# Gautham-JS/ROS_Stereo_SLAM

Hardware: AMD Instinct MI355X
Metric: stereo frames/sec @1241x376, 4096 kpts (higher is better)
Workload: dtype u8/i32 fixed-point (LK) + f32/f64 (geometry)

## Files before the change

### include/svo.h

```cpp
#ifndef SVO_H
#define SVO_H

#include <stddef.h>
#include <stdint.h>

#ifdef __cplusplus
extern "C" {
#endif

#define SVO_VERSION 100

enum {
    SVO_OK = 0,
    SVO_ERR_ARG = -1,
    SVO_ERR_HIP = -2,
    SVO_ERR_CAPACITY = -3,
    SVO_ERR_NO_DEVICE = -4,
    SVO_ERR_TRACKING_LOST = -5,
    SVO_ERR_STATE = -6
};
enum { SVO_MEM_HOST = 0, SVO_MEM_DEVICE = 1 };

enum {
    SVO_K_PYRAMID = 0,
    SVO_K_LK = 1,
    SVO_K_FRANSAC = 2,
    SVO_K_TRIANGULATE = 3,
    SVO_K_PNP = 4,
    SVO_K_POSEGRAPH = 5,
    SVO_K_ANMS = 6,
    SVO_K_BRIEF_INTEGRAL = 7,
    SVO_K_BRIEF_DESCRIBE = 8,
    SVO_K_COUNT = 9
};

typedef struct svo_ctx svo_ctx;
typedef struct svo_pyramid svo_pyramid;
typedef struct svo_vo svo_vo;
typedef struct svo_posegraph svo_posegraph;

int svo_version(void);
const char *svo_last_error(void);

int svo_ctx_create(int device, svo_ctx **out);
int svo_ctx_destroy(svo_ctx *ctx);
int svo_ctx_sync(svo_ctx *ctx);
void *svo_ctx_stream(svo_ctx *ctx);
int svo_ctx_enable_kernel_timing(svo_ctx *ctx, int enable);
int svo_ctx_kernel_time(svo_ctx *ctx, int kernel_id, double *total_ms, int *launches);
int svo_ctx_reset_kernel_time(svo_ctx *ctx);

enum { SVO_MATH_SIN = 0, SVO_MATH_COS = 1, SVO_MATH_ACOS = 2, SVO_MATH_CBRT = 3, SVO_MATH_LOG = 4, SVO_MATH_EXP = 5 };
int svo_math_eval(svo_ctx *ctx, int fn, const double *x, int n, double *y, int mem);

int svo_selftest_fransac_gate(svo_ctx *ctx, const float *d_p1, const float *d_p2, int n, double threshold,
                              uint64_t seed, int lean, uint8_t *d_mask, unsigned *tickets_after);
enum { SVO_SCAN_256_INT = 0, SVO_SCAN_1024_UINT = 1, SVO_SCAN_1024_U64 = 2 };
int svo_selftest_scan(svo_ctx *ctx, int kind, const void *d_in, int n, void *d_out, void *d_total);

int svo_pyramid_create(svo_ctx *ctx, int width, int height, int channels, int levels,
                       svo_pyramid **out);
int svo_pyramid_destroy(svo_ctx *ctx, svo_pyramid *pyr);
int svo_pyramid_build(svo_ctx *ctx, svo_pyramid *pyr, const uint8_t *image, int mem);
int svo_pyramid_is_mono(svo_ctx *ctx, const svo_pyramid *pyr, int *out);
int svo_pyramid_get_level(svo_ctx *ctx, const svo_pyramid *pyr, int level, uint8_t *out,
                          int mem, int *w, int *h);
int svo_pyramid_create2(svo_ctx *ctx, int width, int height, int channels, int levels, int want_deriv,
                        svo_pyramid **out);
int svo_pyramid_get_padded_level(svo_ctx *ctx, const svo_pyramid *pyr, int level, uint8_t *out, int mem,
                                 int *pw, int *ph);
int svo_pyramid_get_derivative_level(svo_ctx *ctx, const svo_pyramid *pyr, int level, int32_t *out, int mem,
                                     int *pw, int *ph);

int svo_grid_keypoints(svo_ctx *ctx, int rows, int cols, int step, float *out_xy, int cap,
                       int mem, int *count);

int svo_lk_track(svo_ctx *ctx, const svo_pyramid *prev, const svo_pyramid *next,
                 const float *prev_pts, int n, float *next_pts, uint8_t *status, float *err,
                 float *min_eig, int mem);

int svo_lk_track_jobs(svo_ctx *ctx, int n_jobs, svo_pyramid *const *prev, const svo_pyramid *const *next,
                      const float *const *d_prev_pts, const int *n, float *const *d_next_pts, uint8_t *const *d_status,
                      float *const *d_err, float *const *d_min_eig, const int *const *d_gates);
int svo_pyramid_build_gated(svo_ctx *ctx, svo_pyramid *pyr, const uint8_t *d_image, const int *d_gate);
int svo_pyramid_build_many(svo_ctx *ctx, int k, svo_pyramid *const *pyrs, const uint8_t *const *d_images,
                           const int *const *d_gates);

int svo_compact(svo_ctx *ctx, const uint8_t *mask, int n, const float *in_a, int stride_a, float *out_a,
                const float *in_b, int stride_b, float *out_b, const float *in_c, int stride_c, float *out_c,
                int *count, int mem);

int svo_fransac(svo_ctx *ctx, const float *p1, const float *p2, int n, double threshold,
                double confidence, int max_iters, uint64_t seed, uint8_t *mask, double *F9,
                int *inlier_count, int *iters_run, int mem);
typedef struct svo_fransac_problem {
    const float *p1, *p2;
    int cap;
    const int *d_n;
    double threshold, confidence;
    int max_iters;
    uint64_t seed;
    uint8_t *mask;
    double *F9;
    int *inlier_count, *iters_run;
    const float *payload_in[3];
    float *payload_out[3];
    int payload_stride[3];
    int *payload_count;
    const int *gate;
} svo_fransac_problem;
int svo_fransac_batch(svo_ctx *ctx, int k, const svo_fransac_problem *problems);

int svo_stereo_projections(double fx, double fy, double cx, double cy, double baseline, double *P1,
                           double *P2);
int svo_triangulate(svo_ctx *ctx, const double *P1, const double *P2, const float *x1, const float *x2,
                    int n, float *out_xyz, float *out_h4, int mem);
int svo_transform_points(svo_ctx *ctx, const double *Rt, const float *in_xyz, int n, float *out_xyz,
                         int mem);
int svo_get_colors(svo_ctx *ctx, const svo_pyramid *pyr, const float *xy, int n, float *out_bgr, int mem);

#define SVO_DEDUP_BOX  0
#define SVO_DEDUP_DISC 1
int svo_dedup_points(svo_ctx *ctx, const float *ref_xy, int n_ref, const int *ref_idx, int n_idx, const float *new_xy,
                     int n_new, double radius, int mode, uint8_t *keep, int *n_keep, int mem);
int svo_replenish(svo_ctx *ctx, float *ref_xy, float *ref_xyz, int n_ref, int cap, const float *new_xy, const float *new_xyz,
// ... 452 lines not shown
```

### ros_stereo_slam_amd/csrc/pyramid.hip

```cpp
#include <cstdlib>

#include "pyr_grey_plan.hip.h"
#include "svo_internal.h"

namespace {

namespace pgp = pyr_grey_plan;

__device__ __forceinline__ int reflect101(int p, int len)
{
    if (len == 1)
        return 0;
    while (p < 0 || p >= len)
        p = p < 0 ? -p : 2 * (len - 1) - p;
    return p;
}

constexpr int TW = 32, TH = 8;
constexpr int PB = 64;
constexpr int SW = 2 * TW + 3, SH = 2 * TH + 3;
constexpr int ROWS_PER_BLOCK = 8;
constexpr int PYR_JOBS = 2 * SVO_LK_MAX_JOBS;

template <int NJ> struct PyrBuildN {
    const uint8_t *img[NJ];
    uint8_t *lvl[NJ][SVO_MAX_LEVELS];
    int *dlvl[NJ];
    const int *gate[NJ];
    int doff[SVO_MAX_LEVELS];
    int pitch[SVO_MAX_LEVELS], dpitch[SVO_MAX_LEVELS], w[SVO_MAX_LEVELS], h[SVO_MAX_LEVELS];
    int levels;
    int gdelta[SVO_MAX_LEVELS], gdoff[SVO_MAX_LEVELS];
    int storage;
};
using PyrBuild = PyrBuildN<PYR_JOBS>;
constexpr int PYR_FEW = 2;
inline PyrBuildN<PYR_FEW> pyr_few(const PyrBuild &b)
{
    PyrBuildN<PYR_FEW> f;
    for (int a = 0; a < PYR_FEW; a++) {
        f.img[a] = b.img[a];
        for (int l = 0; l < SVO_MAX_LEVELS; l++)
            f.lvl[a][l] = b.lvl[a][l];
        f.dlvl[a] = b.dlvl[a];
        f.gate[a] = b.gate[a];
    }
    for (int l = 0; l < SVO_MAX_LEVELS; l++) {
        f.doff[l] = b.doff[l];
        f.pitch[l] = b.pitch[l];
        f.dpitch[l] = b.dpitch[l];
        f.w[l] = b.w[l];
        f.h[l] = b.h[l];
        f.gdelta[l] = b.gdelta[l];
        f.gdoff[l] = b.gdoff[l];
    }
    f.levels = b.levels;
    f.storage = b.storage;
    return f;
}
static_assert(sizeof(PyrBuild) <= 3072, "kernel arguments are limited to 4 KB");
static_assert(pgp::PAD == SVO_PYR_PAD && pgp::LANES == PB && pgp::TILE_W == TW && pgp::TILE_H == TH && pgp::SRC_W == SW &&
                  pgp::SRC_H == SH,
              "pyr_grey_plan.hip.h restates these");

template <int C, bool RAW, int SC = C>
__device__ __forceinline__ void down_tile(const uint8_t *__restrict__ src, int spitch, int w, int h,
                                          uint8_t *__restrict__ dst, int dpitch, int dw, int dh, int tx, int ty)
{
    constexpr int ND = (SW * C + 3) / 4;
    constexpr int SROW = (ND + 1) * 4;
    constexpr int VROW = ND * 4 + 4;
    __shared__ __attribute__((aligned(16))) uint8_t s_src[SH * SROW];
    __shared__ __attribute__((aligned(16))) uint16_t s_v[TH][VROW];
    const int tid = threadIdx.x;
    const int ox = tx * TW, oy = ty * TH;
    const int x0 = 2 * ox - 2, y0 = 2 * oy - 2;
    const bool interior = SC == C && x0 >= 0 && x0 + SW <= w && y0 >= 0 && y0 + SH <= h &&
                          (!RAW || (size_t)(y0 + SH - 1) * spitch + (size_t)x0 * C + (ND + 1) * 4 + 4 <= (size_t)h * spitch);
    bool grey_interior = false;
    if constexpr (RAW && C == 1 && SC == 3) {
        static_assert(ND == pgp::SRC_ND, "the staged row of pyr_grey_plan.hip.h");
        grey_interior = pgp::l1_tile_interior(src, w, h, x0, y0);
    }
    if (grey_interior) {
        if constexpr (RAW && C == 1 && SC == 3) {
            uint32_t staged[pgp::L1_TURNS];
#pragma unroll
            for (int turn = 0; turn < pgp::L1_TURNS; turn++) {
                const int i = min(turn * PB + tid, pgp::L1_ITEMS - 1);
                staged[turn] = pgp::l1_stage_item(src, w, x0, y0, i / ND, i % ND);
            }
#pragma unroll
            for (int turn = 0; turn < pgp::L1_TURNS; turn++) {
                const int i = turn * PB + tid;
                if (i < pgp::L1_ITEMS)
                    reinterpret_cast<uint32_t *>(s_src + (i / ND) * SROW)[i % ND] = staged[turn];
            }
        }
    } else if (interior) {
        for (int d = tid; d < ND; d += PB) {
            const uint8_t *col = src + (ptrdiff_t)y0 * spitch + x0 * C;
#pragma unroll 1
            for (int r = 0; r < SH; r++) {
                const uint8_t *row = col + (ptrdiff_t)r * spitch;
                const unsigned sh = (unsigned)(reinterpret_cast<uintptr_t>(row) & 3);
                const uint32_t *p = reinterpret_cast<const uint32_t *>(row - sh) + d;
                reinterpret_cast<uint32_t *>(s_src + r * SROW)[d] = __builtin_amdgcn_alignbyte(p[1], p[0], sh);
            }
        }
    } else {
        for (int d = tid; d < ND; d += PB) {
            int sx[4];
#pragma unroll
// ... 179 lines not shown

template <int C, int NJ> __global__ __launch_bounds__(PB) void pyr_down_kernel(PyrBuildN<NJ> b, int l)
{
    svo_chain_priority();
    const int job = blockIdx.z;
    if (b.gate[job] && *b.gate[job] == 0)
        return;
    if constexpr (C == 3) {
        if (__builtin_amdgcn_readfirstlane(pyr_words_of(b, job, C)[SVO_PYR_STORED]) == 1) {
            down_tile<1, false>(b.lvl[job][l - 1] + b.gdelta[l - 1], svo_grey_pitch(b.w[l - 1]), b.w[l - 1], b.h[l - 1],
                                b.lvl[job][l] + b.gdelta[l], svo_grey_pitch(b.w[l]), b.w[l], b.h[l], blockIdx.x, blockIdx.y);
            return;
        }
    }
    down_tile<C, false>(b.lvl[job][l - 1], b.pitch[l - 1], b.w[l - 1], b.h[l - 1], b.lvl[job][l], b.pitch[l],
                        b.w[l], b.h[l], blockIdx.x, blockIdx.y);
}

template <int C>
__device__ __forceinline__ void fill_border_row(uint8_t *__restrict__ level, int w, int h, int pitch, int row, int d)
{
    const bool interior_row = row >= SVO_PYR_PAD && row < SVO_PYR_PAD + h;
    const int cb0 = d * 4;
    if (interior_row && cb0 >= SVO_PYR_PAD * C && cb0 + 3 < (SVO_PYR_PAD + w) * C)
        return;
    uint8_t *prow = level + (size_t)row * pitch;
    const int Y = reflect101(row - SVO_PYR_PAD, h);
    const uint8_t *srow = level + (size_t)(Y + SVO_PYR_PAD) * pitch + SVO_PYR_PAD * C;
#pragma unroll
    for (int b = 0; b < 4; b++) {
        int cb = cb0 + b;
        int px = cb / C, ch = cb - px * C;
        bool inside = interior_row && px >= SVO_PYR_PAD && px < SVO_PYR_PAD + w;
        if (inside)
            continue;
        uint8_t v = 0;
        if (px < w + 2 * SVO_PYR_PAD)
            v = srow[reflect101(px - SVO_PYR_PAD, w) * C + ch];
        prow[cb] = v;
    }
}

template <int C> __device__ __forceinline__ bool scharr_edge(int w, int q) { return q == 0 || 4 * q + 4 + C > w * C; }
template <int C> __device__ __forceinline__ void scharr_edge_offsets(int w, int q, int (&off)[12])
{
#pragma unroll
    for (int i = 0; i < 12; i++) {
        const int cb = 4 * q - 4 + i;
        const int px = cb >= 0 ? cb / C : -((-cb + C - 1) / C);
        off[i] = reflect101(px, w) * C + (cb - px * C);
    }
}

template <int C>
__device__ __forceinline__ void scharr_row(const uint8_t *__restrict__ lvl, int *__restrict__ dlvl, int pitch, int dpitch,
                                           int w, int h, int y, int q, const int (&edge_off)[12])
{
    const uint8_t *rows[3] = {lvl + (ptrdiff_t)reflect101(y - 1, h) * pitch, lvl + (ptrdiff_t)y * pitch,
                              lvl + (ptrdiff_t)reflect101(y + 1, h) * pitch};
    uint32_t win[3][3];
    if (!scharr_edge<C>(w, q)) {
#pragma unroll
        for (int r = 0; r < 3; r++) {
            const uint32_t *p = reinterpret_cast<const uint32_t *>(rows[r]) + (q - 1);
            win[r][0] = p[0];
            win[r][1] = p[1];
            win[r][2] = p[2];
        }
    } else {
#pragma unroll
        for (int r = 0; r < 3; r++)
#pragma unroll
            for (int d = 0; d < 3; d++) {
                uint32_t v = 0;
#pragma unroll
                for (int bb = 0; bb < 4; bb++)
                    v |= (uint32_t)rows[r][edge_off[4 * d + bb]] << (8 * bb);
                win[r][d] = v;
            }
    }
    typedef short short2v __attribute__((ext_vector_type(2)));
    short2v S[6], V[6];
#pragma unroll
    for (int k = 0; k < 6; k++) {
        const unsigned sel = (k & 1) ? 0x0c030c02u : 0x0c010c00u;
        const short2v a = __builtin_bit_cast(short2v, __builtin_amdgcn_perm(0u, win[0][k >> 1], sel));
        const short2v bq = __builtin_bit_cast(short2v, __builtin_amdgcn_perm(0u, win[1][k >> 1], sel));
        const short2v c = __builtin_bit_cast(short2v, __builtin_amdgcn_perm(0u, win[2][k >> 1], sel));
        const short2v three = {3, 3}, ten = {10, 10};
        S[k] = (a + c) * three + bq * ten;
        V[k] = c - a;
    }
    auto pair_at = [](const short2v (&P)[6], int pos) -> short2v {
        if ((pos & 1) == 0)
            return P[pos >> 1];
        return __builtin_bit_cast(short2v, __builtin_amdgcn_perm(__builtin_bit_cast(unsigned, P[(pos >> 1) + 1]),
                                                                 __builtin_bit_cast(unsigned, P[pos >> 1]), 0x05040302u));
    };
    int out[4];
#pragma unroll
    for (int j = 0; j < 4; j += 2) {
        const short2v four = {4, 4}, twelve = {12, 12}, forty = {40, 40};
        const short2v dx = (pair_at(S, 4 + C + j) - pair_at(S, 4 - C + j)) * four;
        const short2v dy = (pair_at(V, 4 - C + j) + pair_at(V, 4 + C + j)) * twelve + pair_at(V, 4 + j) * forty;
        const unsigned ux = __builtin_bit_cast(unsigned, dx), uy = __builtin_bit_cast(unsigned, dy);
        out[j] = (int)__builtin_amdgcn_perm(uy, ux, 0x05040100u);
        out[j + 1] = (int)__builtin_amdgcn_perm(uy, ux, 0x07060302u);
    }
    int *drow = reinterpret_cast<int *>(reinterpret_cast<uint8_t *>(dlvl) + (ptrdiff_t)y * dpitch);
    const int rem = w * C - 4 * q;
    if (rem >= 4) {
        typedef int int4v __attribute__((ext_vector_type(4)));
        *reinterpret_cast<int4v *>(drow + 4 * q) = int4v{out[0], out[1], out[2], out[3]};
    } else {
        for (int j = 0; j < rem; j++)
            drow[4 * q + j] = out[j];
    }
}

struct FinishPlan {
    int border_y0[SVO_MAX_LEVELS + 1];
    int scharr_y0[SVO_MAX_LEVELS + 1];
    int publish;
};
template <int S, int NJ, class Pitch, class DPitch>
__device__ __forceinline__ void finish_roles(const PyrBuildN<NJ> &b, const FinishPlan &plan, int job, int by, const int (&ldelta)[SVO_MAX_LEVELS],
                                             const int (&ldoff)[SVO_MAX_LEVELS], Pitch pitch, DPitch dpitch)
{
    if (by < plan.border_y0[b.levels]) {
        int l = 1;
        for (int i = 2; i < b.levels; i++)
            l = by >= plan.border_y0[i] ? i : l;
        const int d = blockIdx.x * PB + threadIdx.x;
        if (d >= (pitch(l) >> 2))
            return;
        uint8_t *padded = b.lvl[job][l] + ldelta[l] - (size_t)SVO_PYR_PAD * pitch(l) - SVO_PYR_PAD * S;
        for (int row = (by - plan.border_y0[l]) * ROWS_PER_BLOCK, rend = min(row + ROWS_PER_BLOCK, b.h[l] + 2 * SVO_PYR_PAD);
             row < rend; row++)
            fill_border_row<S>(padded, b.w[l], b.h[l], pitch(l), row, d);
        return;
    }
    if (!b.dlvl[job])
        return;
    int l = 0;
    for (int i = 1; i < b.levels; i++)
        l = by >= plan.scharr_y0[i] ? i : l;
    const int q = blockIdx.x * PB + threadIdx.x;
    if (4 * q >= b.w[l] * S)
        return;
    int edge_off[12] = {0, 0, 0, 0, 0, 0, 0, 0, 0, 0, 0, 0};
    if (scharr_edge<S>(b.w[l], q))
        scharr_edge_offsets<S>(b.w[l], q, edge_off);
    for (int y = (by - plan.scharr_y0[l]) * ROWS_PER_BLOCK, yend = min(y + ROWS_PER_BLOCK, b.h[l]); y < yend; y++)
        scharr_row<S>(b.lvl[job][l] + ldelta[l], b.dlvl[job] + ldoff[l], pitch(l), dpitch(l), b.w[l], b.h[l], y, q, edge_off);
}

template <int C, int NJ> __global__ __launch_bounds__(PB) void pyr_finish_kernel(PyrBuildN<NJ> b, FinishPlan plan)
{
    svo_chain_priority();
    const int job = blockIdx.z, by = blockIdx.y;
    if (b.gate[job] && *b.gate[job] == 0)
        return;
    if constexpr (C == 3) {
        int *words = pyr_words_of(b, job, C);
        const bool grey = __builtin_amdgcn_readfirstlane(words[SVO_PYR_STORED]) == 1;
        if (blockIdx.x == 0 && by == 0 && threadIdx.x == 0) {
            if (plan.publish) {
                words[SVO_PYR_MONO] = words[SVO_PYR_COLOUR_SEEN] == 0;
                words[SVO_PYR_COLOUR_SEEN] = 0;
                words[SVO_PYR_COLOUR_VALID] = 0;
            } else {
                words[SVO_PYR_COLOUR_VALID] &= ~2;
            }
        }
        if (grey) {
            finish_roles<1>(b, plan, job, by, b.gdelta, b.gdoff, [&](int l) { return svo_grey_pitch(b.w[l]); },
                            [&](int l) { return svo_grey_dpitch(b.w[l]); });
            return;
        }
    }
    const int zero[SVO_MAX_LEVELS] = {0, 0, 0, 0};
    finish_roles<C>(b, plan, job, by, zero, b.doff, [&](int l) { return b.pitch[l]; }, [&](int l) { return b.dpitch[l]; });
}

}

static int alloc_derivative_levels(svo_ctx *ctx, svo_pyramid *p)
{
    size_t ints = 0;
    for (int l = 0; l < p->levels; l++) {
        p->dpitch[l] = (((p->dev.w[l] + 2 * SVO_DERIV_PAD) * p->c * 4 + 15) / 16) * 16;
        const size_t lvl_ints = (size_t)(p->dpitch[l] / 4) * (p->dev.h[l] + 2 * SVO_DERIV_PAD);
        p->doff[l] = ints + (size_t)SVO_DERIV_PAD * (p->dpitch[l] / 4) + (size_t)SVO_DERIV_PAD * p->c;
        ints += (lvl_ints + 63) & ~(size_t)63;
    }
    if (p->c == 3)
        for (int l = 0; l < p->levels; l++) {
            const int gdp = svo_grey_dpitch(p->dev.w[l]);
            p->gdoff[l] = ints + (size_t)SVO_DERIV_PAD * (gdp / 4) + (size_t)SVO_DERIV_PAD;
            ints += ((size_t)(gdp / 4) * (p->dev.h[l] + 2 * SVO_DERIV_PAD) + 63) & ~(size_t)63;
        }
    const size_t dbytes = ints * 4 + 1024;
    hipError_t e = hipMalloc((void **)&p->dbase, dbytes);
    if (e == hipSuccess)
        e = hipMemsetAsync(p->dbase, 0, dbytes, ctx->stream);
    if (e != hipSuccess) {
        (void)hipFree(p->dbase);
        p->dbase = nullptr;
        svo_set_error("hipMalloc derivative levels -> %s", hipGetErrorString(e));
        return SVO_ERR_HIP;
    }
    return SVO_OK;
}

static void fill_build(PyrBuild &b, int k, svo_pyramid *const *pyrs, const uint8_t *const *d_images, bool deriv_only,
                       const int *const *gates = nullptr)
{
    for (int a = 0; a < PYR_JOBS; a++)
        b.gate[a] = gates ? gates[a < k ? a : 0] : nullptr;
    const svo_pyramid *p0 = pyrs[0];
    for (int l = 0; l < SVO_MAX_LEVELS; l++) {
        b.pitch[l] = p0->dev.pitch[l];
        b.w[l] = p0->dev.w[l];
        b.h[l] = p0->dev.h[l];
        b.dpitch[l] = 0;
        b.doff[l] = 0;
        b.gdelta[l] = p0->gdelta[l];
        b.gdoff[l] = 0;
    }
    b.levels = p0->levels;
    static const int mono_storage = getenv("SVO_PYR_MONO_STORAGE") ? atoi(getenv("SVO_PYR_MONO_STORAGE")) : 1;
    b.storage = mono_storage;
    for (int a = 0; a < PYR_JOBS; a++) {
        svo_pyramid *p = pyrs[a < k ? a : 0];
        b.img[a] = d_images ? d_images[a < k ? a : 0] : nullptr;
        for (int l = 0; l < SVO_MAX_LEVELS; l++)
            b.lvl[a][l] = l < p->levels ? const_cast<uint8_t *>(p->dev.lvl[l]) : nullptr;
        const bool d = p->dbase && (deriv_only || p->want_deriv) && (p->c == 1 || p->c == 3);
        b.dlvl[a] = d ? p->dbase : nullptr;
        if (d)
            for (int l = 0; l < SVO_MAX_LEVELS; l++) {
                b.dpitch[l] = p->dpitch[l];
                b.doff[l] = (int)p->doff[l];
                b.gdoff[l] = (int)p->gdoff[l];
            }
    }
}

template <int C> static int launch_finish(svo_ctx *ctx, int k, const PyrBuild &b, bool borders)
{
    FinishPlan plan;
    int y = 0, xmax = 1;
    for (int l = 0; l <= SVO_MAX_LEVELS; l++)
        plan.border_y0[l] = plan.scharr_y0[l] = 0;
    for (int l = 1; l < b.levels; l++) {
        plan.border_y0[l] = y;
        if (borders) {
            y += (b.h[l] + 2 * SVO_PYR_PAD + ROWS_PER_BLOCK - 1) / ROWS_PER_BLOCK;
            xmax = max(xmax, ((b.pitch[l] >> 2) + PB - 1) / PB);
        }
    }
    for (int l = b.levels; l <= SVO_MAX_LEVELS; l++)
        plan.border_y0[l] = y;
    plan.border_y0[b.levels] = y;
    bool any_deriv = false;
    for (int a = 0; a < k; a++)
        any_deriv = any_deriv || b.dlvl[a];
    for (int l = 0; l < b.levels; l++) {
        plan.scharr_y0[l] = y;
        if (any_deriv) {
            y += (b.h[l] + ROWS_PER_BLOCK - 1) / ROWS_PER_BLOCK;
            xmax = max(xmax, ((b.w[l] * C + 3) / 4 + PB - 1) / PB);
        }
    }
    plan.scharr_y0[b.levels] = y;
    plan.publish = borders ? 1 : 0;
    if (y == 0)
        return SVO_OK;
    if (k <= PYR_FEW)
        hipLaunchKernelGGL((pyr_finish_kernel<C, PYR_FEW>), dim3(xmax, y, k), dim3(PB), 0, ctx->stream, pyr_few(b), plan);
    else
        hipLaunchKernelGGL((pyr_finish_kernel<C, PYR_JOBS>), dim3(xmax, y, k), dim3(PB), 0, ctx->stream, b, plan);
    SVO_HIP(hipGetLastError());
    return SVO_OK;
}

int svo_build_derivatives(svo_ctx *ctx, int k, svo_pyramid *const *pyrs)
{
    if (k <= 0)
        return SVO_OK;
    if (k > PYR_JOBS) {
        svo_set_error("pyramid: at most %d per launch", PYR_JOBS);
        return SVO_ERR_ARG;
    }
    for (int a = 0; a < k; a++)
        if (pyrs[a]->c != 1 && pyrs[a]->c != 3) {
            svo_set_error("pyramid: %d channels carry no derivative levels", pyrs[a]->c);
            return SVO_ERR_STATE;
        }
    for (int a = 0; a < k; a++)
        if (!pyrs[a]->dbase) {
            SVO_HIP(hipSetDevice(ctx->device));
            const int rc = alloc_derivative_levels(ctx, pyrs[a]);
            if (rc)
                return rc;
        }
    PyrBuild b;
    fill_build(b, k, pyrs, nullptr, true);
    const int rc = pyrs[0]->c == 1 ? launch_finish<1>(ctx, k, b, false) : launch_finish<3>(ctx, k, b, false);
    if (rc == SVO_OK)
        for (int a = 0; a < k; a++)
            pyrs[a]->has_deriv = true;
    return rc;
}

template <int C>
static int build_levels(svo_ctx *ctx, int k, svo_pyramid *const *pyrs, const uint8_t *const *d_images, const int *const *gates)
{
    PyrBuild b;
    fill_build(b, k, pyrs, d_images, false, gates);
    if constexpr (C == 3) {
        const int quads = (b.w[0] * b.h[0] + 3) / 4, gx = (quads + PB * HEAD_TURNS - 1) / (PB * HEAD_TURNS);
        if (k <= PYR_FEW)
            hipLaunchKernelGGL((pyr_head_kernel<PYR_FEW>), dim3(gx, k), dim3(PB), 0, ctx->stream, pyr_few(b));
        else
            hipLaunchKernelGGL((pyr_head_kernel<PYR_JOBS>), dim3(gx, k), dim3(PB), 0, ctx->stream, b);
    }
    {
        const int tiles_x = b.levels > 1 ? (b.w[1] + TW - 1) / TW : 0, tiles_y = b.levels > 1 ? (b.h[1] + TH - 1) / TH : 0;
        const int n_tiles = tiles_x * tiles_y;
        const int pad_x = ((b.pitch[0] >> 2) + PB - 1) / PB,
                  pad_y = (b.h[0] + 2 * SVO_PYR_PAD + ROWS_PER_BLOCK - 1) / ROWS_PER_BLOCK;
        if (k <= PYR_FEW)
            hipLaunchKernelGGL((pyr_base_kernel<C, PYR_FEW>), dim3(n_tiles + pad_x * pad_y, k), dim3(PB), 0, ctx->stream,
                               pyr_few(b), tiles_x > 0 ? tiles_x : 1, n_tiles, pad_x);
// ... 211 lines not shown
    return svo_pyramid_create_ex(ctx, width, height, channels, levels, want_deriv != 0, out);
}

int svo_pyramid_get_padded_level(svo_ctx *ctx, const svo_pyramid *pyr, int level, uint8_t *out, int mem, int *pw, int *ph)
{
    SVO_CHECK_ARG(ctx && pyr && level >= 0 && level < pyr->levels);
    SVO_CHECK_ARG(mem == SVO_MEM_HOST || mem == SVO_MEM_DEVICE);
    const int W = pyr->dev.w[level] + 2 * SVO_PYR_PAD, H = pyr->dev.h[level] + 2 * SVO_PYR_PAD;
    if (pw)
        *pw = W;
    if (ph)
        *ph = H;
    if (out) {
        const int rc = svo_expand_grey_storage(ctx, pyr, false);
        if (rc)
            return rc;
        const size_t rowb = (size_t)W * pyr->c;
        SVO_HIP(hipMemcpy2DAsync(out, rowb, pyr->base + pyr->off[level], pyr->dev.pitch[level], rowb, H,
                                 mem == SVO_MEM_HOST ? hipMemcpyDeviceToHost : hipMemcpyDeviceToDevice, ctx->stream));
        if (mem == SVO_MEM_HOST)
            SVO_HIP(hipStreamSynchronize(ctx->stream));
    }
    return SVO_OK;
}

int svo_pyramid_get_derivative_level(svo_ctx *ctx, const svo_pyramid *pyr, int level, int32_t *out, int mem, int *pw, int *ph)
{
    SVO_CHECK_ARG(ctx && pyr && level >= 0 && level < pyr->levels);
    SVO_CHECK_ARG(mem == SVO_MEM_HOST || mem == SVO_MEM_DEVICE);
    if (!pyr->dbase || !pyr->has_deriv || (pyr->c != 1 && pyr->c != 3)) {
        svo_set_error("pyramid: holds no derivative levels");
        return SVO_ERR_STATE;
    }
    const int W = pyr->dev.w[level] + 2 * SVO_DERIV_PAD, H = pyr->dev.h[level] + 2 * SVO_DERIV_PAD;
    if (pw)
        *pw = W;
    if (ph)
        *ph = H;
    if (out) {
        const int rc = svo_expand_grey_storage(ctx, pyr, true);
        if (rc)
            return rc;
        const size_t rowb = (size_t)W * pyr->c * sizeof(int32_t);
        const int *first = pyr->dbase + pyr->doff[level] - (size_t)SVO_DERIV_PAD * (pyr->dpitch[level] / 4) -
                           (size_t)SVO_DERIV_PAD * pyr->c;
        SVO_HIP(hipMemcpy2DAsync(out, rowb, first, pyr->dpitch[level], rowb, H,
                                 mem == SVO_MEM_HOST ? hipMemcpyDeviceToHost : hipMemcpyDeviceToDevice, ctx->stream));
        if (mem == SVO_MEM_HOST)
            SVO_HIP(hipStreamSynchronize(ctx->stream));
    }
    return SVO_OK;
}

int svo_pyramid_build_many(svo_ctx *ctx, int k, svo_pyramid *const *pyrs, const uint8_t *const *d_images,
                           const int *const *d_gates)
{
    SVO_CHECK_ARG(ctx && k >= 1 && k <= PYR_JOBS && pyrs && d_images);
    for (int a = 0; a < k; a++)
        SVO_CHECK_ARG(pyrs[a] && d_images[a]);
    return svo_build_pyramids_from_device(ctx, k, pyrs, d_images, d_gates);
}

}
```

### ros_stereo_slam_amd/csrc/svo_internal.h

```cpp
#pragma once

#include <hip/hip_runtime.h>

#include <cstdint>
#include <cstdio>
#include <cstring>
#include <string>
#include <vector>

#include "../../include/svo.h"
#include "../../include/svo_math.h"

#define SVO_MAX_LEVELS 4
#define SVO_LK_WIN 21
#define SVO_PYR_PAD 32
#define SVO_LK_MAX_JOBS 16

#define SVO_N_TICKETS 64
static_assert(32 + 2 * SVO_LK_MAX_JOBS <= SVO_N_TICKETS, "svo_ctx::d_tickets: lk_expand_kernel's slots end past the allocation");

void svo_set_error(const char *fmt, ...);

__device__ __forceinline__ void svo_chain_priority() { __builtin_amdgcn_s_setprio(3); }

// ... 17 lines not shown
    } while (0)

struct PyrDev {
    const uint8_t *lvl[SVO_MAX_LEVELS];
    int pitch[SVO_MAX_LEVELS];
    int w[SVO_MAX_LEVELS];
    int h[SVO_MAX_LEVELS];
    int levels;
    int c;
};

struct Mat34 {
    double m[12];
};

#define SVO_PYR_HEADER 256
enum { SVO_PYR_MONO = 0, SVO_PYR_COLOUR_SEEN = 1, SVO_PYR_STORED = 2, SVO_PYR_COLOUR_VALID = 3 };
__host__ __device__ __forceinline__ int *svo_pyr_words(const uint8_t *padded)
{
    return reinterpret_cast<int *>(const_cast<uint8_t *>(padded) - SVO_PYR_HEADER);
}
__host__ __device__ __forceinline__ int svo_grey_pitch(int w) { return (w + 2 * SVO_PYR_PAD + 15) & ~15; }
__host__ __device__ __forceinline__ int svo_grey_dpitch(int w) { return ((w + 2 * 32 ) * 4 + 15) & ~15; }
__device__ __forceinline__ const uint8_t *svo_pyr_pixel0(const uint8_t *lvl0, int pitch, int c, int w, int gdelta0, int x, int y,
                                                         int *step)
{
    *step = c >= 3 ? 1 : 0;
    if (c == 3) {
        const int *words = svo_pyr_words(lvl0 - (ptrdiff_t)SVO_PYR_PAD * pitch - SVO_PYR_PAD * c);
        if (words[SVO_PYR_STORED] == 1) {
            *step = 0;
            return lvl0 + gdelta0 + (ptrdiff_t)y * svo_grey_pitch(w) + x;
        }
    }
    return lvl0 + (size_t)y * pitch + x * c;
}

struct svo_pyramid {
    int w, h, c, levels;
    uint8_t *base;
    size_t off[SVO_MAX_LEVELS];
    uint8_t *origin(int l) const
    {
        return base + off[l] + (size_t)SVO_PYR_PAD * dev.pitch[l] + (size_t)SVO_PYR_PAD * c;
    }
    size_t bytes;
    PyrDev dev;
    int *dbase = nullptr;
    size_t doff[SVO_MAX_LEVELS] = {0, 0, 0, 0};
    int dpitch[SVO_MAX_LEVELS] = {0, 0, 0, 0};
    size_t goff[SVO_MAX_LEVELS] = {0, 0, 0, 0}, gdoff[SVO_MAX_LEVELS] = {0, 0, 0, 0};
    int gdelta[SVO_MAX_LEVELS] = {0, 0, 0, 0};
    bool want_deriv = true, has_deriv = false;
};
#define SVO_DERIV_PAD 32
int svo_build_derivatives(svo_ctx *ctx, int k, svo_pyramid *const *pyrs);
int svo_expand_grey_storage(svo_ctx *ctx, const svo_pyramid *pyr, bool deriv);
int svo_pyramid_create_ex(svo_ctx *ctx, int width, int height, int channels, int levels, bool want_deriv,
                          svo_pyramid **out);

struct DevBuf {
    void *p = nullptr;
    size_t cap = 0;
    int ensure(size_t bytes);
    void release();
    template <class T> T *as() { return reinterpret_cast<T *>(p); }
};

struct KernelTimer {
    std::vector<std::pair<hipEvent_t, hipEvent_t>> pending;
    std::vector<std::pair<hipEvent_t, hipEvent_t>> pool;
    double total_ms = 0;
    int launches = 0;
};

struct svo_ctx {
    int device = 0;
    hipStream_t stream = nullptr;
    bool timing = false;
    KernelTimer timers[SVO_K_COUNT];
    DevBuf s_img, s_a, s_b, s_c, s_d, s_e, s_f, s_g;
    DevBuf w_a, w_b, w_c, w_d, w_e;
    unsigned *d_tickets = nullptr;
    void *pinned = nullptr;
    size_t pinned_bytes = 0;
    hipEvent_t wait_ev = nullptr;
    struct svo_orb *orb_cache = nullptr;
    int orb_key[5] = {0, 0, 0, 0, 0};
    DevBuf orb_out;
    std::vector<unsigned char> orb_host;
    struct svo_orb_cv *orb_cv_cache = nullptr;
    int orb_cv_key[8] = {0, 0, 0, 0, 0, 0, 0, 0};
    int8_t orb_pattern[1024];
    int has_pattern = 0;
    DevBuf orb_cv_out, orb_cv_img, orb_cv_ptrs;
    hipStream_t up_stream = nullptr;
    DevBuf up_ring;
    hipEvent_t up_ev[3] = {nullptr, nullptr, nullptr}, use_ev[3] = {nullptr, nullptr, nullptr};
    DevBuf sgbm_cost, sgbm_misc, sgbm_rp;
    DevBuf bm_work;
    DevBuf sor_grid;
    DevBuf icp_work;
    DevBuf ess;
    DevBuf feat_img, feat_sum;
    DevBuf sift_pyr, sift_work, sift_out;
    DevBuf brief_work, brief_pat;
// ... 220 lines not shown
```

Measured before the change: 14670.

## Flatten pyramid finish kernel into a balanced 1D work-item schedule with row-reuse Scharr

Replaces the 3D grid (x blocks × per-level row bands × jobs) of the pyramid finish kernel with a 1D grid. A host-built plan packs border-fill and Scharr items per job and spreads them evenly across workgroups, and grey-stored pyramids pick a row granularity that fits the same workgroup count. The Scharr pass now processes several rows per thread with a rolling three-row window, so each source row is loaded once instead of three times. This is meant to remove idle blocks in the old rectangular grid and redundant loads, at the cost of a larger kernel argument and per-item decode logic. The change also adds a small public accessor for a pyramid's device memory regions.

```diff
diff --git a/include/svo.h b/include/svo.h
--- a/include/svo.h
+++ b/include/svo.h
@@ -71,6 +71,7 @@
                                  int *pw, int *ph);
 int svo_pyramid_get_derivative_level(svo_ctx *ctx, const svo_pyramid *pyr, int level, int32_t *out, int mem,
                                      int *pw, int *ph);
+int svo_pyramid_device_regions(const svo_pyramid *pyr, void **base, size_t *bytes, void **dbase, size_t *dbytes);
 
 int svo_grid_keypoints(svo_ctx *ctx, int rows, int cols, int step, float *out_xy, int cap,
                        int mem, int *count);
diff --git a/ros_stereo_slam_amd/csrc/pyr_finish_plan.hip.h b/ros_stereo_slam_amd/csrc/pyr_finish_plan.hip.h
--- /dev/null
+++ b/ros_stereo_slam_amd/csrc/pyr_finish_plan.hip.h
@@ -0,0 +1,140 @@
+#pragma once
+
+#if defined(__HIPCC__)
+#define PYR_FINISH_HD __host__ __device__ inline __attribute__((always_inline))
+#else
+#define PYR_FINISH_HD inline
+#endif
+
+namespace pyr_finish_plan {
+
+constexpr int PAD = 32;
+constexpr int LANES = 64;
+constexpr int MAX_LEVELS = 4;
+constexpr int MAX_JOBS = 32;
+constexpr int ROWS = 8;
+enum { BORDER = 0, SCHARR = 1 };
+
+struct Table {
+    int S;
+    int rows;
+    int n[2];
+    int start[2][MAX_LEVELS];
+    int xb[2][MAX_LEVELS];
+    int ext_x[2][MAX_LEVELS];
+    int ext_rows[2][MAX_LEVELS];
+};
+
+struct Item {
+    int role, level;
+    int row0, nrows;
+    int x0, nx;
+};
+
+struct Plan {
+    Table full, grey;
+    int has_grey;
+    int k, nd;
+    int nbw, nsw;
+    unsigned dmask;
+    int publish;
+    unsigned char djob[MAX_JOBS];
+};
+
+PYR_FINISH_HD int pitch_of(int w, int S) { return ((w + 2 * PAD) * S + 15) / 16 * 16; }
+PYR_FINISH_HD int ceil_div(int a, int b) { return (a + b - 1) / b; }
+
+inline Table make_table(int levels, const int *w, const int *h, int S, int rows, bool borders, bool scharr)
+{
+    Table t;
+    t.S = S;
+    t.rows = rows;
+    for (int role = 0; role < 2; role++) {
+        int n = 0;
+        for (int l = 0; l < MAX_LEVELS; l++) {
+            const bool has = l < levels && (role == BORDER ? borders && l >= 1 : scharr);
+            t.start[role][l] = n;
+            t.ext_x[role][l] = !has ? 0 : role == BORDER ? pitch_of(w[l], S) / 4 : (w[l] * S + 3) / 4;
+            t.ext_rows[role][l] = !has ? 0 : role == BORDER ? h[l] + 2 * PAD : h[l];
+            t.xb[role][l] = has ? ceil_div(t.ext_x[role][l], LANES) : 1;
+            n += has ? t.xb[role][l] * ceil_div(t.ext_rows[role][l], rows) : 0;
+        }
+        t.n[role] = n;
+    }
+    return t;
+}
+
+PYR_FINISH_HD int job_items(const Table &t, bool deriv) { return t.n[BORDER] + (deriv ? t.n[SCHARR] : 0); }
+PYR_FINISH_HD int job_wgs(const Plan &p, bool deriv) { return p.nbw + (deriv ? p.nsw : 0); }
+PYR_FINISH_HD int grid_wgs(const Plan &p) { return p.k * p.nbw + p.nd * p.nsw; }
+
+inline Plan make_plan(int levels, const int *w, const int *h, int C, bool borders, int k, const bool *deriv)
+{
+    Plan p;
+    p.k = k;
+    p.nd = 0;
+    p.dmask = 0;
+    p.publish = borders ? 1 : 0;
+    for (int a = 0; a < MAX_JOBS; a++)
+        p.djob[a] = 0;
+    for (int a = 0; a < k; a++)
+        if (deriv[a]) {
+            p.dmask |= 1u << a;
+            p.djob[p.nd++] = (unsigned char)a;
+        }
+    p.full = make_table(levels, w, h, C, ROWS, borders, p.nd > 0);
+    p.nsw = p.full.n[SCHARR];
+    p.nbw = p.full.n[BORDER];
+    if (borders && p.nbw == 0 && p.nsw > 0)
+        p.nbw = 1;
+    p.has_grey = C == 3;
+    p.grey = p.full;
+    if (p.has_grey)
+        for (int rows = 1; rows <= ROWS; rows++) {
+            p.grey = make_table(levels, w, h, 1, rows, borders, p.nd > 0);
+            if (job_items(p.grey, false) <= job_wgs(p, false) && (p.nd == 0 || job_items(p.grey, true) <= job_wgs(p, true)))
+                break;
+        }
+    return p;
+}
+
+PYR_FINISH_HD void decode(const Plan &p, int wg, int *job, int *i, bool *deriv)
+{
+    const int first = p.k * p.nbw;
+    if (wg < first) {
+        *job = wg / p.nbw;
+        *i = wg - *job * p.nbw;
+        *deriv = (p.dmask >> *job) & 1u;
+    } else {
+        const int r = wg - first, j = r / p.nsw;
+        *job = p.djob[j];
+        *i = p.nbw + (r - j * p.nsw);
+        *deriv = true;
+    }
+}
+
+PYR_FINISH_HD void run(int items, int n_wg, int i, int *begin, int *end)
+{
+    const int per = ceil_div(items, n_wg);
+    *begin = i * per < items ? i * per : items;
+    *end = *begin + per < items ? *begin + per : items;
+}
+
+PYR_FINISH_HD Item item_of(const Table &t, int idx)
+{
+    Item it;
+    it.role = idx < t.n[BORDER] ? BORDER : SCHARR;
+    const int i = idx - (it.role == SCHARR ? t.n[BORDER] : 0);
+    int l = 0;
+    for (int m = 1; m < MAX_LEVELS; m++)
+        l = i >= t.start[it.role][m] ? m : l;
+    it.level = l;
+    const int j = i - t.start[it.role][l], rb = j / t.xb[it.role][l], xbi = j - rb * t.xb[it.role][l];
+    it.row0 = rb * t.rows;
+    it.nrows = t.ext_rows[it.role][l] - it.row0 < t.rows ? t.ext_rows[it.role][l] - it.row0 : t.rows;
+    it.x0 = xbi * LANES;
+    it.nx = t.ext_x[it.role][l] - it.x0 < LANES ? t.ext_x[it.role][l] - it.x0 : LANES;
+    return it;
+}
+
+}
diff --git a/ros_stereo_slam_amd/csrc/pyramid.hip b/ros_stereo_slam_amd/csrc/pyramid.hip
--- a/ros_stereo_slam_amd/csrc/pyramid.hip
+++ b/ros_stereo_slam_amd/csrc/pyramid.hip
@@ -1,11 +1,13 @@
 #include <cstdlib>
 
+#include "pyr_finish_plan.hip.h"
 #include "pyr_grey_plan.hip.h"
 #include "svo_internal.h"
 
 namespace {
 
 namespace pgp = pyr_grey_plan;
+namespace pfp = pyr_finish_plan;
 
 __device__ __forceinline__ int reflect101(int p, int len)
 {
@@ -58,7 +60,10 @@
     f.storage = b.storage;
     return f;
 }
-static_assert(sizeof(PyrBuild) <= 3072, "kernel arguments are limited to 4 KB");
+static_assert(sizeof(PyrBuild) + sizeof(pfp::Plan) <= 3584, "kernel arguments are limited to 4 KB");
+static_assert(pfp::PAD == SVO_PYR_PAD && pfp::LANES == PB && pfp::MAX_LEVELS == SVO_MAX_LEVELS && pfp::MAX_JOBS == PYR_JOBS &&
+                  pfp::ROWS == ROWS_PER_BLOCK,
+              "pyr_finish_plan.hip.h restates these");
 static_assert(pgp::PAD == SVO_PYR_PAD && pgp::LANES == PB && pgp::TILE_W == TW && pgp::TILE_H == TH && pgp::SRC_W == SW &&
                   pgp::SRC_H == SH,
               "pyr_grey_plan.hip.h restates these");
@@ -344,44 +349,24 @@
     }
 }
 
-template <int C>
-__device__ __forceinline__ void scharr_row(const uint8_t *__restrict__ lvl, int *__restrict__ dlvl, int pitch, int dpitch,
-                                           int w, int h, int y, int q, const int (&edge_off)[12])
-{
-    const uint8_t *rows[3] = {lvl + (ptrdiff_t)reflect101(y - 1, h) * pitch, lvl + (ptrdiff_t)y * pitch,
-                              lvl + (ptrdiff_t)reflect101(y + 1, h) * pitch};
-    uint32_t win[3][3];
-    if (!scharr_edge<C>(w, q)) {
-#pragma unroll
-        for (int r = 0; r < 3; r++) {
-            const uint32_t *p = reinterpret_cast<const uint32_t *>(rows[r]) + (q - 1);
-            win[r][0] = p[0];
-            win[r][1] = p[1];
-            win[r][2] = p[2];
-        }
-    } else {
-#pragma unroll
-        for (int r = 0; r < 3; r++)
-#pragma unroll
-            for (int d = 0; d < 3; d++) {
-                uint32_t v = 0;
-#pragma unroll
-                for (int bb = 0; bb < 4; bb++)
-                    v |= (uint32_t)rows[r][edge_off[4 * d + bb]] << (8 * bb);
-                win[r][d] = v;
-            }
-    }
-    typedef short short2v __attribute__((ext_vector_type(2)));
-    short2v S[6], V[6];
+typedef short short2v __attribute__((ext_vector_type(2)));
+__device__ __forceinline__ void scharr_unpack(const uint32_t (&raw)[3], short2v (&u)[6])
+{
 #pragma unroll
     for (int k = 0; k < 6; k++) {
         const unsigned sel = (k & 1) ? 0x0c030c02u : 0x0c010c00u;
-        const short2v a = __builtin_bit_cast(short2v, __builtin_amdgcn_perm(0u, win[0][k >> 1], sel));
-        const short2v bq = __builtin_bit_cast(short2v, __builtin_amdgcn_perm(0u, win[1][k >> 1], sel));
-        const short2v c = __builtin_bit_cast(short2v, __builtin_amdgcn_perm(0u, win[2][k >> 1], sel));
+        u[k] = __builtin_bit_cast(short2v, __builtin_amdgcn_perm(0u, raw[k >> 1], sel));
+    }
+}
+template <int C>
+__device__ __forceinline__ void scharr_store(const short2v (&a)[6], const short2v (&bq)[6], const short2v (&c)[6], int *drow, int q, int rem)
+{
+    short2v S[6], V[6];
+#pragma unroll
+    for (int k = 0; k < 6; k++) {
         const short2v three = {3, 3}, ten = {10, 10};
-        S[k] = (a + c) * three + bq * ten;
-        V[k] = c - a;
+        S[k] = (a[k] + c[k]) * three + bq[k] * ten;
+        V[k] = c[k] - a[k];
     }
     auto pair_at = [](const short2v (&P)[6], int pos) -> short2v {
         if ((pos & 1) == 0)
@@ -399,8 +384,6 @@
         out[j] = (int)__builtin_amdgcn_perm(uy, ux, 0x05040100u);
         out[j + 1] = (int)__builtin_amdgcn_perm(uy, ux, 0x07060302u);
     }
-    int *drow = reinterpret_cast<int *>(reinterpret_cast<uint8_t *>(dlvl) + (ptrdiff_t)y * dpitch);
-    const int rem = w * C - 4 * q;
     if (rem >= 4) {
         typedef int int4v __attribute__((ext_vector_type(4)));
         *reinterpret_cast<int4v *>(drow + 4 * q) = int4v{out[0], out[1], out[2], out[3]};
@@ -410,53 +393,134 @@
     }
 }
 
-struct FinishPlan {
-    int border_y0[SVO_MAX_LEVELS + 1];
-    int scharr_y0[SVO_MAX_LEVELS + 1];
-    int publish;
-};
+template <int C, int N>
+__device__ __forceinline__ void scharr_rows(const uint8_t *__restrict__ lvl, int *__restrict__ dlvl, int pitch, int dpitch,
+                                            int w, int h, int y0, int q)
+{
+    uint32_t win[N + 2][3];
+#pragma unroll
+    for (int r = 0; r < N + 2; r++) {
+        const uint32_t *p = reinterpret_cast<const uint32_t *>(lvl + (ptrdiff_t)reflect101(y0 - 1 + r, h) * pitch) + (q - 1);
+        win[r][0] = p[0];
+        win[r][1] = p[1];
+        win[r][2] = p[2];
+    }
+    short2v U[3][6];
+    scharr_unpack(win[0], U[0]);
+    scharr_unpack(win[1], U[1]);
+#pragma unroll
+    for (int r = 0; r < N; r++) {
+        scharr_unpack(win[r + 2], U[(r + 2) % 3]);
+        scharr_store<C>(U[r % 3], U[(r + 1) % 3], U[(r + 2) % 3],
+                        reinterpret_cast<int *>(reinterpret_cast<uint8_t *>(dlvl) + (ptrdiff_t)(y0 + r) * dpitch), q, w * C - 4 * q);
+    }
+}
+template <int C>
+__device__ __forceinline__ void scharr_rows_mixed(const uint8_t *__restrict__ lvl, int *__restrict__ dlvl, int pitch, int dpitch,
+                                                  int w, int h, int y0, int n, int q, bool edge, const int (&edge_off)[12])
+{
+    auto load_row = [&](int y, uint32_t (&raw)[3]) {
+        const uint8_t *row = lvl + (ptrdiff_t)reflect101(y, h) * pitch;
+        if (!edge) {
+            const uint32_t *p = reinterpret_cast<const uint32_t *>(row) + (q - 1);
+            raw[0] = p[0];
+            raw[1] = p[1];
+            raw[2] = p[2];
+        } else {
+#pragma unroll
+            for (int d = 0; d < 3; d++) {
+                uint32_t v = 0;
+#pragma unroll
+                for (int bb = 0; bb < 4; bb++)
+                    v |= (uint32_t)row[edge_off[4 * d + bb]] << (8 * bb);
+                raw[d] = v;
+            }
+        }
+    };
+    short2v a[6] = {}, bq[6] = {}, c[6] = {};
+    uint32_t next[3];
+    load_row(y0 - 1, next);
+#pragma unroll 1
+    for (int r = -2; r < n; r++) {
+        const uint32_t raw[3] = {next[0], next[1], next[2]};
+        if (r + 1 < n)
+            load_row(y0 + r + 2, next);
+#pragma unroll
+        for (int k = 0; k < 6; k++) {
+            a[k] = bq[k];
+            bq[k] = c[k];
+        }
+        scharr_unpack(raw, c);
+        if (r >= 0)
+            scharr_store<C>(a, bq, c, reinterpret_cast<int *>(reinterpret_cast<uint8_t *>(dlvl) + (ptrdiff_t)(y0 + r) * dpitch), q,
+                            w * C - 4 * q);
+    }
+}
+
 template <int S, int NJ, class Pitch, class DPitch>
-__device__ __forceinline__ void finish_roles(const PyrBuildN<NJ> &b, const FinishPlan &plan, int job, int by, const int (&ldelta)[SVO_MAX_LEVELS],
-                                             const int (&ldoff)[SVO_MAX_LEVELS], Pitch pitch, DPitch dpitch)
-{
-    if (by < plan.border_y0[b.levels]) {
-        int l = 1;
-        for (int i = 2; i < b.levels; i++)
-            l = by >= plan.border_y0[i] ? i : l;
-        const int d = blockIdx.x * PB + threadIdx.x;
-        if (d >= (pitch(l) >> 2))
-            return;
-        uint8_t *padded = b.lvl[job][l] + ldelta[l] - (size_t)SVO_PYR_PAD * pitch(l) - SVO_PYR_PAD * S;
-        for (int row = (by - plan.border_y0[l]) * ROWS_PER_BLOCK, rend = min(row + ROWS_PER_BLOCK, b.h[l] + 2 * SVO_PYR_PAD);
-             row < rend; row++)
-            fill_border_row<S>(padded, b.w[l], b.h[l], pitch(l), row, d);
-        return;
-    }
-    if (!b.dlvl[job])
-        return;
-    int l = 0;
-    for (int i = 1; i < b.levels; i++)
-        l = by >= plan.scharr_y0[i] ? i : l;
-    const int q = blockIdx.x * PB + threadIdx.x;
-    if (4 * q >= b.w[l] * S)
-        return;
-    int edge_off[12] = {0, 0, 0, 0, 0, 0, 0, 0, 0, 0, 0, 0};
-    if (scharr_edge<S>(b.w[l], q))
-        scharr_edge_offsets<S>(b.w[l], q, edge_off);
-    for (int y = (by - plan.scharr_y0[l]) * ROWS_PER_BLOCK, yend = min(y + ROWS_PER_BLOCK, b.h[l]); y < yend; y++)
-        scharr_row<S>(b.lvl[job][l] + ldelta[l], b.dlvl[job] + ldoff[l], pitch(l), dpitch(l), b.w[l], b.h[l], y, q, edge_off);
-}
-
-template <int C, int NJ> __global__ __launch_bounds__(PB) void pyr_finish_kernel(PyrBuildN<NJ> b, FinishPlan plan)
+__device__ __forceinline__ void finish_items(const PyrBuildN<NJ> &b, const pfp::Table &T, int job, bool deriv, int n_wg, int i,
+                                             const int (&ldelta)[SVO_MAX_LEVELS], const int (&ldoff)[SVO_MAX_LEVELS], Pitch pitch,
+                                             DPitch dpitch)
+{
+    int t0, t1;
+    pfp::run(pfp::job_items(T, deriv), n_wg, i, &t0, &t1);
+    for (int t = t0; t < t1; t++) {
+        const pfp::Item it = pfp::item_of(T, t);
+        const bool active = (int)threadIdx.x < it.nx;
+        const int l = it.level, x = it.x0 + threadIdx.x;
+        if (it.role == pfp::BORDER) {
+            if (!active)
+                continue;
+            uint8_t *padded = b.lvl[job][l] + ldelta[l] - (size_t)SVO_PYR_PAD * pitch(l) - SVO_PYR_PAD * S;
+            for (int row = it.row0; row < it.row0 + it.nrows; row++)
+                fill_border_row<S>(padded, b.w[l], b.h[l], pitch(l), row, x);
+            continue;
+        }
+        const uint8_t *lvl = b.lvl[job][l] + ldelta[l];
+        int *dl = b.dlvl[job] + ldoff[l];
+        const bool edge = active && scharr_edge<S>(b.w[l], x);
+        if (__builtin_amdgcn_ballot_w64(edge) != 0) {
+            if (active) {
+                int edge_off[12] = {0, 0, 0, 0, 0, 0, 0, 0, 0, 0, 0, 0};
+                if (edge)
+                    scharr_edge_offsets<S>(b.w[l], x, edge_off);
+                scharr_rows_mixed<S>(lvl, dl, pitch(l), dpitch(l), b.w[l], b.h[l], it.row0, it.nrows, x, edge, edge_off);
+            }
+            continue;
+        }
+        if (!active)
+            continue;
+        switch (it.nrows) {
+#define SCHARR_CASE(N)                                                               \
+    case N:                                                                          \
+        scharr_rows<S, N>(lvl, dl, pitch(l), dpitch(l), b.w[l], b.h[l], it.row0, x); \
+        break;
+            SCHARR_CASE(1)
+            SCHARR_CASE(2)
+            SCHARR_CASE(3)
+            SCHARR_CASE(4)
+            SCHARR_CASE(5)
+            SCHARR_CASE(6)
+            SCHARR_CASE(7)
+            SCHARR_CASE(8)
+#undef SCHARR_CASE
+        }
+    }
+}
+
+template <int C, int NJ> __global__ __launch_bounds__(PB) void pyr_finish_kernel(PyrBuildN<NJ> b, pfp::Plan plan)
 {
     svo_chain_priority();
-    const int job = blockIdx.z, by = blockIdx.y;
+    int job, i;
+    bool deriv;
+    pfp::decode(plan, blockIdx.x, &job, &i, &deriv);
     if (b.gate[job] && *b.gate[job] == 0)
         return;
+    const int n_wg = pfp::job_wgs(plan, deriv);
     if constexpr (C == 3) {
         int *words = pyr_words_of(b, job, C);
         const bool grey = __builtin_amdgcn_readfirstlane(words[SVO_PYR_STORED]) == 1;
-        if (blockIdx.x == 0 && by == 0 && threadIdx.x == 0) {
+        if (i == 0 && threadIdx.x == 0) {
             if (plan.publish) {
                 words[SVO_PYR_MONO] = words[SVO_PYR_COLOUR_SEEN] == 0;
                 words[SVO_PYR_COLOUR_SEEN] = 0;
@@ -466,13 +530,13 @@
             }
         }
         if (grey) {
-            finish_roles<1>(b, plan, job, by, b.gdelta, b.gdoff, [&](int l) { return svo_grey_pitch(b.w[l]); },
+            finish_items<1>(b, plan.grey, job, deriv, n_wg, i, b.gdelta, b.gdoff, [&](int l) { return svo_grey_pitch(b.w[l]); },
                             [&](int l) { return svo_grey_dpitch(b.w[l]); });
             return;
         }
     }
     const int zero[SVO_MAX_LEVELS] = {0, 0, 0, 0};
-    finish_roles<C>(b, plan, job, by, zero, b.doff, [&](int l) { return b.pitch[l]; }, [&](int l) { return b.dpitch[l]; });
+    finish_items<C>(b, plan.full, job, deriv, n_wg, i, zero, b.doff, [&](int l) { return b.pitch[l]; }, [&](int l) { return b.dpitch[l]; });
 }
 
 }
@@ -502,6 +566,7 @@
         svo_set_error("hipMalloc derivative levels -> %s", hipGetErrorString(e));
         return SVO_ERR_HIP;
     }
+    p->dbytes = dbytes;
     return SVO_OK;
 }
 
@@ -541,38 +606,17 @@
 
 template <int C> static int launch_finish(svo_ctx *ctx, int k, const PyrBuild &b, bool borders)
 {
-    FinishPlan plan;
-    int y = 0, xmax = 1;
-    for (int l = 0; l <= SVO_MAX_LEVELS; l++)
-        plan.border_y0[l] = plan.scharr_y0[l] = 0;
-    for (int l = 1; l < b.levels; l++) {
-        plan.border_y0[l] = y;
-        if (borders) {
-            y += (b.h[l] + 2 * SVO_PYR_PAD + ROWS_PER_BLOCK - 1) / ROWS_PER_BLOCK;
-            xmax = max(xmax, ((b.pitch[l] >> 2) + PB - 1) / PB);
-        }
-    }
-    for (int l = b.levels; l <= SVO_MAX_LEVELS; l++)
-        plan.border_y0[l] = y;
-    plan.border_y0[b.levels] = y;
-    bool any_deriv = false;
-    for (int a = 0; a < k; a++)
-        any_deriv = any_deriv || b.dlvl[a];
-    for (int l = 0; l < b.levels; l++) {
-        plan.scharr_y0[l] = y;
-        if (any_deriv) {
-            y += (b.h[l] + ROWS_PER_BLOCK - 1) / ROWS_PER_BLOCK;
-            xmax = max(xmax, ((b.w[l] * C + 3) / 4 + PB - 1) / PB);
-        }
-    }
-    plan.scharr_y0[b.levels] = y;
-    plan.publish = borders ? 1 : 0;
-    if (y == 0)
+    bool deriv[PYR_JOBS];
+    for (int a = 0; a < PYR_JOBS; a++)
+        deriv[a] = a < k && b.dlvl[a];
+    const pfp::Plan plan = pfp::make_plan(b.levels, b.w, b.h, C, borders, k, deriv);
+    const int n_wg = pfp::grid_wgs(plan);
+    if (n_wg == 0)
         return SVO_OK;
     if (k <= PYR_FEW)
-        hipLaunchKernelGGL((pyr_finish_kernel<C, PYR_FEW>), dim3(xmax, y, k), dim3(PB), 0, ctx->stream, pyr_few(b), plan);
+        hipLaunchKernelGGL((pyr_finish_kernel<C, PYR_FEW>), dim3(n_wg), dim3(PB), 0, ctx->stream, pyr_few(b), plan);
     else
-        hipLaunchKernelGGL((pyr_finish_kernel<C, PYR_JOBS>), dim3(xmax, y, k), dim3(PB), 0, ctx->stream, b, plan);
+        hipLaunchKernelGGL((pyr_finish_kernel<C, PYR_JOBS>), dim3(n_wg), dim3(PB), 0, ctx->stream, b, plan);
     SVO_HIP(hipGetLastError());
     return SVO_OK;
 }
@@ -890,6 +934,16 @@
     return SVO_OK;
 }
 
+int svo_pyramid_device_regions(const svo_pyramid *pyr, void **base, size_t *bytes, void **dbase, size_t *dbytes)
+{
+    SVO_CHECK_ARG(pyr && base && bytes && dbase && dbytes);
+    *base = pyr->base;
+    *bytes = pyr->bytes;
+    *dbase = pyr->dbase;
+    *dbytes = pyr->dbase ? pyr->dbytes : 0;
+    return SVO_OK;
+}
+
 int svo_pyramid_build_many(svo_ctx *ctx, int k, svo_pyramid *const *pyrs, const uint8_t *const *d_images,
                            const int *const *d_gates)
 {
diff --git a/ros_stereo_slam_amd/csrc/svo_internal.h b/ros_stereo_slam_amd/csrc/svo_internal.h
--- a/ros_stereo_slam_amd/csrc/svo_internal.h
+++ b/ros_stereo_slam_amd/csrc/svo_internal.h
@@ -93,6 +93,7 @@
     size_t goff[SVO_MAX_LEVELS] = {0, 0, 0, 0}, gdoff[SVO_MAX_LEVELS] = {0, 0, 0, 0};
     int gdelta[SVO_MAX_LEVELS] = {0, 0, 0, 0};
     bool want_deriv = true, has_deriv = false;
+    size_t dbytes = 0;
 };
 #define SVO_DERIV_PAD 32
 int svo_build_derivatives(svo_ctx *ctx, int k, svo_pyramid *const *pyrs);
```

Result: no change. 14800 (median of 6 runs) (+0.8%).
